# Lacadame/DiffSci

Measured on AMD Instinct MI355X. Metric: samples/sec (50-step Karras Heun), PUNetG 64ch 128x128, higher is better.
Workload: dtype f32 (3x3 convs: fp16 hi+lo split, 3 fp16 MFMA products, fp32 accumulate); 1 GPU; PUNetG 64-base-ch, 1x128x128 fields, batch 64 per GPU, 50-step Heun deterministic sampler (99 network evaluations); global_batch=64, parallelism=dp1 (batch shards, all-gather of samples), world_size=1, backend=none (one process), hipgraph=True

## Files before the change

diffsci_amd/_native.py:

```python
import ctypes
import os
from ctypes import POINTER, Structure, c_char_p, c_float, c_int, c_longlong, c_size_t, c_uint32, c_uint64, c_void_p

_HERE = os.path.dirname(os.path.abspath(__file__))
LIB_PATH = os.environ.get("DIFFSCI_HIP_LIB") or os.path.join(_HERE, "_lib", "libdiffsci_hip.so")

ABI_VERSION = 4
DS_IN_NETWORK, DS_IN_SCORE, DS_IN_DRIFT, DS_IN_FLOW = 0, 1, 2, 3
DS_LOAD_PLAIN, DS_LOAD_MAXPOOL2, DS_LOAD_UPSAMPLE2, DS_LOAD_AVGPOOL2 = 0, 1, 2, 3
DS_PAD_CIRCULAR = 16
DS_RES1_UPSAMPLED = 32


class EvalCoef(Structure):
    _fields_ = [("c_out", c_float), ("c_skip", c_float), ("sigma_sq", c_float),
                ("neg_mult", c_float), ("neg_lang", c_float), ("guidance", c_float),
                ("one_minus_guidance", c_float), ("input_kind", c_int), ("stochastic", c_int),
                ("scaled", c_int), ("scale", c_float), ("scale_mult", c_float), ("next_scale", c_float), ("xin_copies", c_int),
                ("nonfinite", c_void_p)]


class NativeLibraryError(RuntimeError):
    pass


_P = c_void_p
_PROTOS = {
    "ds_version": (c_int, []),
    "ds_last_error": (c_char_p, []),
    "ds_device_info": (c_int, [POINTER(c_int), POINTER(c_int), ctypes.c_char_p, c_int]),
    "ds_karras_scale": (c_int, [_P, _P, c_float, c_size_t, _P]),
    "ds_karras_drift": (c_int, [_P, _P, _P, _P, POINTER(EvalCoef), c_size_t, _P]),
    "ds_karras_score": (c_int, [_P, _P, _P, _P, POINTER(EvalCoef), c_size_t, _P]),
    "ds_philox_normal": (c_int, [_P, _P, c_uint64, c_size_t, _P]),
    "ds_karras_euler": (c_int, [_P, _P, _P, _P, _P, POINTER(EvalCoef), c_float, c_float,
                                _P, _P, c_uint64, c_float, c_float, c_size_t, _P]),
    "ds_karras_heun": (c_int, [_P, _P, _P, _P, _P, POINTER(EvalCoef), _P, _P, POINTER(EvalCoef),
                               c_float, c_float, c_size_t, _P]),
    "ds_karras_churn": (c_int, [_P, _P, _P, _P, _P, c_uint64, c_float, c_float, c_float, c_float, c_int, c_size_t, _P]),
    "ds_karras_denoiser": (c_int, [_P, _P, _P, _P, c_float, c_float, _P, _P, c_int, c_size_t, _P]),
    "ds_inorm_silu": (c_int, [_P, _P, _P, _P, c_int, c_int, c_int, c_float, c_int, _P]),
    "ds_conv2d_packed_floats": (c_size_t, [c_int, c_int, c_int]),
    "ds_conv2d_pack_weights": (c_int, [_P, _P, c_int, c_int, c_int, _P]),
    "ds_conv2d": (c_int, [_P, _P, _P, _P, _P, c_int, _P, _P, c_int, c_int, c_int, c_int, c_int,
                          c_int, c_int, _P]),
    "ds_conv2d_x6_packed_bytes": (c_size_t, [c_int, c_int]),
    "ds_conv2d_x6_pack_weights": (c_int, [_P, _P, c_int, c_int, _P]),
    "ds_conv2d_x6": (c_int, [_P, _P, _P, _P, _P, c_int, _P, _P, c_int, c_int, c_int, c_int, c_int, c_int, _P]),
    "ds_conv2d_h3_packed_bytes": (c_size_t, [c_int, c_int]),
    "ds_conv2d_h3_pack_weights": (c_int, [_P, _P, c_int, c_int, c_int, _P]),
    "ds_conv2d_h3": (c_int, [_P, _P, _P, c_int, _P, _P, c_int, _P, _P, c_int, c_int, c_int, c_int, c_int, c_int, _P, _P, _P, _P, _P]),
    "ds_absmax_rows": (c_int, [_P, _P, c_int, c_size_t, c_size_t, _P]),
    "ds_amax_merge": (c_int, [_P, _P, _P, c_int, _P]),
    "ds_absmax_channels": (c_int, [_P, _P, _P, _P, _P, c_int, c_int, c_size_t, c_int, _P]),
    "ds_input_amax": (c_int, [_P, c_int, c_int, _P, _P, _P, c_int, c_int, c_size_t, c_int, _P]),
    "ds_fill_u32": (c_int, [_P, c_uint32, c_size_t, _P]),
    "ds_conv2d_h3_up_supported": (c_int, [c_int, c_int]),
    "ds_conv2d_h3_up_packed_bytes": (c_size_t, [c_int, c_int]),
    "ds_conv2d_h3_up_pack_weights": (c_int, [_P, _P, c_int, c_int, c_int, _P]),
    "ds_conv2d_h3_up": (c_int, [_P, _P, _P, c_int, _P, _P, c_int, _P, _P, c_int, c_int, c_int, c_int, c_int, c_int, _P, _P, _P, _P, _P]),
    "ds_table_apply_images": (c_int, [_P, _P, _P, c_int, c_int, c_int, c_int, _P]),
    "ds_conv2d_h3_up_img": (c_int, [_P, _P, _P, c_int, _P, _P, c_int, _P, _P, c_int, c_int, c_int, c_int, c_int, _P, _P, _P]),
    "ds_conv_tile_count": (c_int, [c_int, c_int]),
    "ds_inorm_table": (c_int, [_P, _P, _P, _P, c_int, c_int, c_int, c_int, c_float, c_int, _P]),
    "ds_gnorm1_table": (c_int, [_P, _P, c_int, c_int, _P, c_int, c_int, _P, _P, _P, _P, c_int, c_int, c_longlong,
                                c_float, c_int, _P]),
    "ds_gnorm1_stats_tiles": (c_int, [_P, _P, c_int, c_int, _P, c_int, c_int, c_int, c_longlong, c_float, c_int, _P]),
    "ds_conv2d_direct": (c_int, [_P, _P, _P, _P, c_int, c_int, c_int, c_int, c_int, c_int, _P]),
    "ds_conv3d_direct": (c_int, [_P, _P, _P, _P, _P, c_int, _P, _P, c_int, c_int, c_int, c_int, c_int, c_int, c_int, _P]),
    "ds_volume_to_slices": (c_int, [_P, _P, c_int, c_int, c_int, c_size_t, c_int, c_int, c_int, _P]),
    "ds_slices_to_volume": (c_int, [_P, _P, _P, _P, c_int, c_int, c_int, c_size_t, c_int, _P]),
    "ds_conv_images_bytes": (c_size_t, [c_int, c_int, c_int, c_int]),
    "ds_inorm_silu_images_supported": (c_int, [c_int, c_int]),
    "ds_inorm_silu_images": (c_int, [_P, _P, _P, _P, c_int, c_int, c_int, c_int, c_float, c_int, _P]),
    "ds_conv2d_h3_img": (c_int, [_P, _P, _P, c_int, _P, _P, c_int, _P, _P, c_int, c_int, c_int, c_int, c_int, c_int, _P, _P, _P]),
    "ds_gnorm1_apply_images": (c_int, [_P, _P, _P, _P, _P, _P, _P, c_int, c_int, c_int, c_int, c_int, c_int, c_int, _P]),
    "ds_volume_stat_tiles": (c_int, [c_int, c_size_t]),
    "ds_volume_to_slices_act": (c_int, [_P, _P, _P, c_int, c_int, c_int, c_size_t, c_int, _P]),
    "ds_wrap_pad_slices": (c_int, [_P, c_int, c_int, c_int, c_size_t, _P]),
    "ds_slices_to_volume_stats": (c_int, [_P, _P, _P, _P, _P, c_int, c_int, c_int, c_size_t, c_int, _P]),
    "ds_slice_tables": (c_int, [_P, _P, _P, _P, c_int, c_int, c_int, c_int, c_longlong, c_float, c_int, c_int, _P]),
    "ds_avgpool3d": (c_int, [_P, _P, c_int, c_int, c_int, c_int, _P]),
    "ds_upsample3d": (c_int, [_P, _P, c_int, c_int, c_int, c_int, _P]),
    "ds_avgpool3d_f": (c_int, [_P, _P, c_int, c_int, c_int, c_int, c_int, _P]),
    "ds_upsample_f": (c_int, [_P, _P, c_int, c_int, c_int, c_int, c_int, c_int, _P]),
    "ds_maxpool_f": (c_int, [_P, _P, c_int, c_int, c_int, c_int, c_int, c_int, _P]),
    "ds_cornerpool_f": (c_int, [_P, _P, _P, _P, c_int, c_int, c_int, c_int, c_int, c_int, c_int, c_int, c_int, _P]),
    "ds_conv1x1_h3_packed_bytes": (c_size_t, [c_int, c_int]),
    "ds_conv1x1_h3_pack_weights": (c_int, [_P, _P, c_int, c_int, c_int, _P]),
    "ds_conv1x1_h3": (c_int, [_P, _P, _P, c_int, _P, _P, c_int, _P, _P, c_int, c_int, c_int, c_int, c_int, c_int, _P, _P, _P, c_int, _P]),
    "ds_attention": (c_int, [_P, _P, c_int, c_int, c_int, _P]),
    "ds_attention_generic": (c_int, [_P, _P, c_int, c_int, c_int, _P]),
    "ds_attention_h3": (c_int, [_P, _P, c_int, c_int, c_int, _P, _P, _P]),
    "ds_attention_h3_workspace_bytes": (c_size_t, [c_int, c_int, c_int]),
    "ds_attention_h3_ws": (c_int, [_P, _P, _P, c_int, c_int, c_int, _P, _P, _P]),
    "ds_attention_h3_heads_workspace_bytes": (c_size_t, [c_int, c_int, c_int, c_int]),
    "ds_attention_h3_heads": (c_int, [_P, _P, _P, c_int, c_int, c_int, c_int, _P, _P, _P]),
    "ds_attention_heads_generic": (c_int, [_P, _P, c_int, c_int, c_int, c_int, _P]),
    "ds_token_l2_normalize": (c_int, [_P, c_int, c_int, c_int, c_int, c_int, c_float, c_float, _P]),
    "ds_linear": (c_int, [_P, _P, _P, _P, c_int, c_int, c_int, c_int, _P]),
    "ds_fourier_features": (c_int, [_P, _P, _P, _P, c_int, c_int, c_int, _P]),
    "ds_fourier_channels": (c_int, [_P, _P, _P, c_int, c_int, c_int, c_size_t, _P]),
    "ds_gnorm1_workspace_bytes": (c_size_t, [c_int]),
    "ds_gnorm1_stats": (c_int, [_P, _P, _P, c_int, c_int, c_int, c_float, c_int, _P]),
    "ds_groupnorm_stats": (c_int, [_P, _P, _P, c_int, c_int, c_int, c_int, c_float, _P]),
    "ds_groupnorm_apply": (c_int, [_P, _P, _P, _P, _P, c_int, c_int, c_int, c_int, c_int, _P, _P]),
    "ds_groupnorm_stats_tiles": (c_int, [_P, _P, c_int, c_int, c_int, c_int, c_longlong, c_float, _P]),
    "ds_groupnorm_table": (c_int, [_P, _P, _P, _P, _P, c_int, c_int, c_int, c_int, c_longlong, c_float, _P]),
    "ds_gnorm1_apply": (c_int, [_P, _P, _P, _P, _P, _P, _P, c_int, c_int, c_int, c_int, c_int, c_int, c_int, _P]),
    "ds_gnorm1_apply_poolf": (c_int, [_P, _P, _P, _P, _P, _P, _P, c_int, c_int, c_int, c_int, c_int, c_int, c_int, _P]),
    "ds_concat2": (c_int, [_P, _P, _P, c_int, c_size_t, c_size_t, _P]),
    "ds_add_act": (c_int, [_P, _P, _P, c_int, c_int, c_int, c_int, _P]),
    "ds_mask_blend": (c_int, [_P, _P, _P, _P, c_size_t, c_int, _P]),
    "ds_axpby": (c_int, [_P, _P, c_float, _P, c_float, c_size_t, _P]),
    "ds_div_scalar": (c_int, [_P, _P, c_float, c_size_t, _P]),
    "ds_batchnorm_eval": (c_int, [_P, _P, _P, _P, _P, _P, c_float, c_float, c_int, c_int, c_int, c_int, c_size_t, _P]),
    "ds_lerp_stack": (c_int, [_P, _P, _P, c_int, c_size_t, _P]),
    "ds_add": (c_int, [_P, _P, _P, c_size_t, _P]),
    "ds_token_layernorm": (c_int, [_P, _P, _P, _P, _P, _P, c_int, c_int, c_int, c_int, c_float, _P, _P]),
    "ds_token_gate": (c_int, [_P, _P, _P, _P, c_int, c_int, c_int, c_int, _P]),
    "ds_silu_amax": (c_int, [_P, _P, c_int, c_size_t, _P, _P]),
    "ds_patch_embed": (c_int, [_P, _P, _P, _P, c_int, c_int, c_int, c_int, c_int, c_int, _P]),
    "ds_patch_unembed": (c_int, [_P, _P, _P, _P, c_int, c_int, c_int, c_int, c_int, c_int, _P]),
    "ds_graph_begin_capture": (c_int, [_P]),
    "ds_graph_end_capture": (c_int, [_P, POINTER(_P), POINTER(c_int)]),
    "ds_graph_launch": (c_int, [_P, _P]),
    "ds_graph_destroy": (c_int, [_P]),
}

_lib = None


def exported_symbols():
    return sorted(_PROTOS)


def lib():
    global _lib
    if _lib is not None:
        return _lib
    if not os.path.exists(LIB_PATH):
        raise NativeLibraryError(
            f"{LIB_PATH} is missing: diffsci_amd has no CPU or PyTorch fallback. "
# ... 23 lines not shown
```

diffsci_amd/csrc/ds_conv1h.hip:

```cpp
#include "ds_common.h"
#include "ds_conv_epilogue.h"

namespace {

using ds_epi::f32x16;
typedef unsigned u32x4 __attribute__((ext_vector_type(4)));
typedef _Float16 f16x8 __attribute__((ext_vector_type(8)));
typedef _Float16 f16x2 __attribute__((ext_vector_type(2)));
typedef const __attribute__((address_space(1))) float* gfloat_ptr;
typedef const __attribute__((address_space(1))) char* gchar_ptr;
typedef float f32x2 __attribute__((ext_vector_type(2)));
typedef const __attribute__((address_space(1))) f32x2* gfloat2_ptr;

constexpr int COT = 64, NT = 256, KC = 16;
constexpr int NPOS = 256;
constexpr int XBUF_VEC = 2 * 2 * NPOS;
constexpr int WSLAB_VEC = 2 * 2 * COT;
constexpr int NXB = 3, NWS = 3;
constexpr int RING_BYTES = (NXB * XBUF_VEC + NWS * WSLAB_VEC) * 16;
constexpr int EPI_BYTES = 4 * 64 * 2 * 32 * 4;
constexpr int STAGE_BYTES = RING_BYTES > EPI_BYTES ? RING_BYTES : EPI_BYTES;
constexpr int LDS_BYTES = STAGE_BYTES + 128 * 4;
constexpr int TWO_RING_BYTES = (NXB * XBUF_VEC + NWS * 2 * WSLAB_VEC) * 16;
constexpr int TWO_EPI_BYTES = 8 * 64 * 2 * 32 * 4;
static_assert(TWO_EPI_BYTES >= TWO_RING_BYTES, "bias / shift rows behind the larger of the two");
constexpr int LDS_BYTES_TWO = TWO_EPI_BYTES + 2 * 128 * 4;
constexpr int NXCD = 8;

struct Conv1hArgs {
  float* out;
  const float* in;
  const u32x4* wp;
  const float* bias;
  const float* shift;
  const float* res1;
  const float* res2;
  float* tile_stats;
  int res1_up;
  const unsigned* in_amax;
  unsigned* out_amax;
  int wshift;
  int amax_split;
  int shift_stride;
  int B, Cin, Cout, H, W, Hin, Win;
  int tiles_x, tiles_y, n_cot, n_chunks;
  int n_cot_wg;
  unsigned n_blocks;
};

__device__ __forceinline__ void split2(float a, float b, unsigned& hi, unsigned& lo) {
  f16x2 h = {(_Float16)a, (_Float16)b};
  unsigned hp = __builtin_bit_cast(unsigned, h);
  asm volatile("" : "+v"(hp));
  const f16x2 hq = __builtin_bit_cast(f16x2, hp);
  f16x2 l = {(_Float16)(a - (float)hq[0]), (_Float16)(b - (float)hq[1])};
  hi = hp;
  lo = __builtin_bit_cast(unsigned, l);
}

__device__ __forceinline__ void step_barrier() {
  asm volatile("s_waitcnt lgkmcnt(0)\n\ts_barrier" ::: "memory");
}

template <int MODE, bool W16, bool TWO = false>
__global__ __launch_bounds__(TWO ? 2 * NT : NT, 2) void k_conv1h(const Conv1hArgs a) {
  constexpr int TW = W16 ? 16 : 32, TH = W16 ? 16 : 8;
  constexpr int COTS = TWO ? 2 : 1;
  constexpr int KR = TWO ? KC / 2 : KC;
  extern __shared__ __attribute__((aligned(16))) unsigned char smem[];
  u32x4* Xs = reinterpret_cast<u32x4*>(smem);
  u32x4* Ws = Xs + NXB * XBUF_VEC;
  float* BS = reinterpret_cast<float*>(smem + (TWO ? TWO_EPI_BYTES : STAGE_BYTES));
  const int tid = threadIdx.x;
  const int lane = tid & 63;
  const int wv = __builtin_amdgcn_readfirstlane(tid >> 6);
  const int cw = TWO ? wv >> 2 : 0;
  const int wq = wv & 3;
  const int pix = tid & (NT - 1);
  const int li = lane & 31, lh = lane >> 5;
// ... 101 lines not shown
  w_fetch(W1, n > 1 ? 1 : 0);
  x_fetch(R1, n > 1 ? 1 : 0);
  __builtin_amdgcn_sched_barrier(0);
  ascale = ds_epi::act_scale_of(amax_bits, a.wshift);
  w_store(W0, 0);
  x_store(R0, 0);
  ds_epi::commit_bias_shift(BS, bias_shift, COTS);
  __syncthreads();

  int buf = 0;
  auto step = [&](float (&Ra)[KR], u32x4& Wa, float (&Rb)[KR], u32x4& Wb, int g) {
    const int gf = g + 2 < n ? g + 2 : n - 1;
    w_fetch(Wa, gf);
    x_fetch(Ra, gf);
    mma(g % NWS, buf);
    const int nb = buf == NXB - 1 ? 0 : buf + 1;
    w_store(Wb, (g + 1) % NWS);
    x_store(Rb, nb);
    buf = nb;
    step_barrier();
  };
  int g = 0;
  for (; g + 1 < n; g += 2) {
    step(R0, W0, R1, W1, g);
    step(R1, W1, R0, W0, g + 1);
  }
  if (g < n) step(R0, W0, R1, W1, g);
  __syncthreads();

  {
    ds_epi::Args e;
    e.out = a.out; e.bias = a.bias; e.shift = a.shift; e.res1 = a.res1; e.res2 = a.res2; e.res1_up = a.res1_up;
    e.unscale = ds_epi::unscale_from_in(ascale.in_scale, a.wshift); e.shift_stride = a.shift_stride;
    e.out_amax = a.out_amax ? a.out_amax + b + ((a.amax_split > 0 && (cot + cw) * COT >= a.amax_split) ? a.B : 0) : nullptr;
    e.b = b; e.co_base = (cot + cw) * COT; e.y0 = y0 + (W16 ? 4 : 2) * wq; e.x0 = x0;
    e.Cout = a.Cout; e.H = a.H; e.W = a.W;
    e.tile_stats = a.tile_stats; e.tile = ty * a.tiles_x + tx; e.ntiles = a.tiles_x * a.tiles_y;
    float* tile = reinterpret_cast<float*>(smem) + wv * (64 * 2 * 32);
    ds_epi::store_tile<W16>(acc, tile, BS + 128 * cw, e);
    if (a.tile_stats) {
      __syncthreads();
      if constexpr (TWO) {
        if (tid < 128) {
          e.co_base = (cot + (tid >> 6)) * COT;
          ds_epi::store_tile_stats(reinterpret_cast<const float*>(smem) + (tid >> 6) * 4 * (64 * 2 * 32), 64 * 2 * 32, e, tid & 63);
        }
      } else {
        ds_epi::store_tile_stats(reinterpret_cast<const float*>(smem), 64 * 2 * 32, e);
      }
    }
  }
}

__global__ void k_pack1h(_Float16* packed, const float* __restrict__ w, int Cout, int Cin, int n_chunks, float scale,
                         size_t total) {
  size_t i = (size_t)blockIdx.x * blockDim.x + threadIdx.x;
  if (i >= total) return;
  size_t t = i;
  const int c8 = t % 8; t /= 8;
  const int co64 = t % COT; t /= COT;
  const int h = t % 2; t /= 2;
  const int piece = t % 2; t /= 2;
  const int chunk = t % n_chunks; t /= n_chunks;
  const int cot = (int)t;
  const int co = cot * COT + co64, ci = chunk * KC + 8 * h + c8;
  float v = 0.f;
  if (co < Cout && ci < Cin) v = w[(size_t)co * Cin + ci] * scale;
  const _Float16 hi = (_Float16)v;
  const _Float16 lo = (_Float16)(v - (float)hi);
  packed[i] = piece == 0 ? hi : lo;
}

inline int conv1h_two() {
  static const int v = [] { const char* e = getenv("DS_CONV1_TWO"); return e ? atoi(e) : 1; }();
  return v;
}
inline long long conv1h_two_min() {
  static const long long v = [] { const char* e = getenv("DS_CONV1_TWO_MIN"); return e ? atoll(e) : 256ll; }();
  return v;
}

template <int MODE, bool W16>
int launch_conv1h(Conv1hArgs a, hipStream_t s) {
  const int two = conv1h_two();
  if (a.n_cot % 2 == 0 && ((two == 1 && (long long)a.n_blocks / 2 >= conv1h_two_min()) || two == 2)) {
    const int rc = ds::ensure_dynamic_lds<&k_conv1h<MODE, W16, true>>((int)(LDS_BYTES_TWO), "hipFuncSetAttribute(conv1h two)");
    if (rc != DS_OK) return rc;
    a.n_cot_wg = a.n_cot / 2;
    a.n_blocks /= 2;
    hipLaunchKernelGGL((k_conv1h<MODE, W16, true>), dim3(a.n_blocks), dim3(2 * NT), LDS_BYTES_TWO, s, a);
    DS_CHECK_LAUNCH("ds_conv1x1_h3");
    return DS_OK;
  }
  {
    const int rc = ds::ensure_dynamic_lds<&k_conv1h<MODE, W16>>((int)(LDS_BYTES), "hipFuncSetAttribute(conv1h)");
    if (rc != DS_OK) return rc;
  }
  a.n_cot_wg = a.n_cot;
  hipLaunchKernelGGL((k_conv1h<MODE, W16>), dim3(a.n_blocks), dim3(NT), LDS_BYTES, s, a);
  DS_CHECK_LAUNCH("ds_conv1x1_h3");
  return DS_OK;
}

}

extern "C" {

size_t ds_conv1x1_h3_packed_bytes(int Cout, int Cin) {
  if (Cout <= 0 || Cin <= 0) return 0;
  const size_t n_cot = (Cout + COT - 1) / COT, n_chunks = (Cin + KC - 1) / KC;
  return n_cot * n_chunks * (size_t)WSLAB_VEC * 16;
}

int ds_conv1x1_h3_pack_weights(void* packed, const float* w, int Cout, int Cin, int wshift, void* stream) {
  DS_REQUIRE(packed && w, DS_ERR_NULL, "ds_conv1x1_h3_pack_weights: NULL pointer");
  DS_REQUIRE(Cout > 0 && Cin > 0, DS_ERR_SHAPE, "ds_conv1x1_h3_pack_weights: Cout=%d Cin=%d", Cout, Cin);
  DS_REQUIRE(wshift >= -40 && wshift <= 40, DS_ERR_SHAPE, "ds_conv1x1_h3_pack_weights: wshift %d out of range", wshift);
  const int n_chunks = (Cin + KC - 1) / KC;
  const size_t total = ds_conv1x1_h3_packed_bytes(Cout, Cin) / 2;
  hipLaunchKernelGGL(k_pack1h, dim3((unsigned)((total + 255) / 256)), dim3(256), 0, ds::as_stream(stream),
                     reinterpret_cast<_Float16*>(packed), w, Cout, Cin, n_chunks, ldexpf(1.0f, wshift), total);
  DS_CHECK_LAUNCH("ds_conv1x1_h3_pack_weights");
  return DS_OK;
}

int ds_conv1x1_h3(float* out, const float* in, const void* w_packed, int wshift, const float* bias, const float* shift,
                  int shift_stride, const float* res1, const float* res2, int B, int Cin, int Cout, int H, int W,
                  int load_mode, float* tile_stats, const unsigned* in_amax, unsigned* out_amax, int amax_split, void* stream) {
  DS_REQUIRE(out && in && w_packed, DS_ERR_NULL, "ds_conv1x1_h3: NULL pointer");
  DS_REQUIRE(B >= 0 && Cin > 0 && Cout > 0 && H > 0 && W > 0, DS_ERR_SHAPE,
             "ds_conv1x1_h3: bad shape B=%d Cin=%d Cout=%d H=%d W=%d", B, Cin, Cout, H, W);
  DS_REQUIRE(load_mode == DS_LOAD_PLAIN || load_mode == DS_LOAD_UPSAMPLE2 || load_mode == DS_LOAD_AVGPOOL2,
             DS_ERR_UNSUPPORTED, "ds_conv1x1_h3: load_mode %d", load_mode);
  DS_REQUIRE(load_mode != DS_LOAD_UPSAMPLE2 || (H % 2 == 0 && W % 2 == 0), DS_ERR_SHAPE,
             "ds_conv1x1_h3: UPSAMPLE2 needs even output H, W (got %d x %d)", H, W);
  DS_REQUIRE(shift == nullptr || shift_stride == 0 || shift_stride >= Cout, DS_ERR_SHAPE,
             "ds_conv1x1_h3: shift_stride %d < Cout %d", shift_stride, Cout);
  DS_REQUIRE((reinterpret_cast<uintptr_t>(w_packed) & 15u) == 0, DS_ERR_SHAPE, "ds_conv1x1_h3: w_packed must be 16-byte aligned");
  DS_REQUIRE(load_mode != DS_LOAD_AVGPOOL2 || (reinterpret_cast<uintptr_t>(in) & 7u) == 0, DS_ERR_SHAPE,
             "ds_conv1x1_h3: AVGPOOL2 input must be 8-byte aligned");
  DS_REQUIRE(wshift >= -40 && wshift <= 40, DS_ERR_SHAPE, "ds_conv1x1_h3: wshift %d out of range", wshift);
  DS_REQUIRE(amax_split >= 0 && amax_split % COT == 0, DS_ERR_SHAPE, "ds_conv1x1_h3: amax_split %d must be a multiple of 64", amax_split);
  if (B == 0) return DS_OK;
  Conv1hArgs a;
  a.out = out; a.in = in; a.wp = reinterpret_cast<const u32x4*>(w_packed); a.bias = bias; a.shift = shift;
  a.res1 = res1; a.res2 = res2; a.shift_stride = shift_stride; a.tile_stats = tile_stats; a.res1_up = 0;
  a.wshift = wshift; a.in_amax = in_amax; a.out_amax = out_amax; a.amax_split = amax_split;
  a.B = B; a.Cin = Cin; a.Cout = Cout; a.H = H; a.W = W;
  a.Hin = load_mode == DS_LOAD_AVGPOOL2 ? 2 * H : (load_mode == DS_LOAD_UPSAMPLE2 ? H / 2 : H);
  a.Win = load_mode == DS_LOAD_AVGPOOL2 ? 2 * W : (load_mode == DS_LOAD_UPSAMPLE2 ? W / 2 : W);
  DS_REQUIRE((long long)a.Hin * a.Win < (1ll << 29), DS_ERR_SHAPE, "ds_conv1x1_h3: a channel plane exceeds 2^29 floats");
  const long long pad32 = (long long)((W + 31) / 32 * 32) * ((H + 7) / 8 * 8);
  const long long pad16 = (long long)((W + 15) / 16 * 16) * ((H + 15) / 16 * 16);
  const bool w16 = pad16 < pad32;
  const int TW = w16 ? 16 : 32, TH = w16 ? 16 : 8;
  a.tiles_x = (W + TW - 1) / TW; a.tiles_y = (H + TH - 1) / TH;
  a.n_cot = (Cout + COT - 1) / COT;
  a.n_chunks = (Cin + KC - 1) / KC;
  const long long blocks = (long long)B * a.tiles_y * a.tiles_x * a.n_cot;
  DS_REQUIRE(blocks > 0 && blocks < (1ll << 31), DS_ERR_SHAPE, "ds_conv1x1_h3: grid of %lld workgroups is out of range", blocks);
  a.n_blocks = (unsigned)blocks;
  hipStream_t s = ds::as_stream(stream);
  if (w16) {
    if (load_mode == DS_LOAD_PLAIN) return launch_conv1h<DS_LOAD_PLAIN, true>(a, s);
    if (load_mode == DS_LOAD_UPSAMPLE2) return launch_conv1h<DS_LOAD_UPSAMPLE2, true>(a, s);
    return launch_conv1h<DS_LOAD_AVGPOOL2, true>(a, s);
  }
  if (load_mode == DS_LOAD_PLAIN) return launch_conv1h<DS_LOAD_PLAIN, false>(a, s);
  if (load_mode == DS_LOAD_UPSAMPLE2) return launch_conv1h<DS_LOAD_UPSAMPLE2, false>(a, s);
  return launch_conv1h<DS_LOAD_AVGPOOL2, false>(a, s);
}

}
```

diffsci_amd/ops.py:

```python
import ctypes

import torch

from . import _native as N
from ._native import EvalCoef


def require_device(t, what="tensor"):
    if not isinstance(t, torch.Tensor):
        raise TypeError(f"{what} must be a torch.Tensor")
    if not t.is_cuda:
        raise RuntimeError(
            f"{what} lives on {t.device}: diffsci_amd computes only on an AMD GPU through "
            "libdiffsci_hip.so (there is no CPU path; move the module and inputs to 'cuda').")
    if t.dtype != torch.float32:
        raise TypeError(f"{what} has dtype {t.dtype}; the HIP path is fp32 only")
    if t.device.index != torch.cuda.current_device():
        raise RuntimeError(f"{what} lives on {t.device} but the current device is cuda:{torch.cuda.current_device()}: "
                           "wrap the call in `with torch.cuda.device(tensor.device):` (KarrasModule / SIModule / the "
                           "networks do this for their own entry points)")


def on_device_of(t):
    return torch.cuda.device(t.device)
# ... 858 lines not shown
def conv_tile_count(H, W):
    return N.lib().ds_conv_tile_count(int(H), int(W))


def table_channels(C):
    return (C + 15) // 16 * 16


def inorm_table(tile_stats, w, b, kind, count, eps=1e-5, out=None):
    B, C, nt, _ = tile_stats.shape
    if out is None:
        out = torch.empty((B, table_channels(C), 4), dtype=torch.float32, device=tile_stats.device)
    elif tuple(out.shape) != (B, table_channels(C), 4):
        raise ValueError(f"table must be {(B, table_channels(C), 4)}")
    N.check(N.lib().ds_inorm_table(_p(out), _p(tile_stats), _p(w), _p(b), B, C, nt, int(count), float(eps), int(kind),
                                   _stream()), "ds_inorm_table")
    return out


def gnorm1_table(stats_a, w, b, kind, count, stats_b=None, film=None, eps=1e-5, out=None):
    B, Ca, nta, _ = stats_a.shape
    Cb, ntb = (0, 0) if stats_b is None else (stats_b.shape[1], stats_b.shape[2])
    C = Ca + Cb
    if out is None:
        out = torch.empty((B, table_channels(C), 4), dtype=torch.float32, device=stats_a.device)
    elif tuple(out.shape) != (B, table_channels(C), 4):
        raise ValueError(f"table must be {(B, table_channels(C), 4)}")
    f1 = f2 = None
    stride = 0
    if film is not None:
        if film.dim() != 2 or film.shape[1] != 2 * C or film.shape[0] not in (1, B):
            raise ValueError("film must be [1 or B, 2C]")
        require_device(film, "film")
        stride = 0 if film.shape[0] == 1 else 2 * C
        f1, f2 = film.data_ptr(), film.data_ptr() + 4 * C
    N.check(N.lib().ds_gnorm1_table(_p(out), _p(stats_a), Ca, nta, _p(stats_b), Cb, ntb, _p(w), _p(b), f1, f2, stride,
                                    B, int(count), float(eps), int(kind), _stream()), "ds_gnorm1_table")
    return out


def gnorm1_stats_tiles(stats_a, kind, count, stats_b=None, eps=1e-5, stats=None):
    require_device(stats_a, "stats_a")
    B, Ca, nta, _ = stats_a.shape
    Cb, ntb = (0, 0) if stats_b is None else (stats_b.shape[1], stats_b.shape[2])
    if stats is None:
        stats = torch.empty((B, 2), dtype=torch.float32, device=stats_a.device)
    elif tuple(stats.shape) != (B, 2):
        raise ValueError(f"stats must be {(B, 2)}")
    N.check(N.lib().ds_gnorm1_stats_tiles(_p(stats), _p(stats_a), Ca, nta, _p(stats_b), Cb, ntb, B, int(count), float(eps),
                                          int(kind), _stream()), "ds_gnorm1_stats_tiles")
    return stats


def conv2d(x, w_packed, Cout, ks, bias=None, shift=None, res1=None, res2=None,
           load_mode=N.DS_LOAD_PLAIN, out=None, kind="fp32", wshift=0, prenorm=None, tile_stats=None, circular=False,
           res1_upsampled=False, w_up=None, up_wshift=0, tap_offset=None, in_amax=None, out_amax=None, amax_split=0):
    B, Cin, Hin, Win = x.shape
    if load_mode in (N.DS_LOAD_MAXPOOL2, N.DS_LOAD_AVGPOOL2):
        if Hin % 2 or Win % 2:
            raise ValueError("pooling load needs even input H, W")
        if (load_mode == N.DS_LOAD_AVGPOOL2) != (kind == "fp16x3" and ks == 1):
            raise ValueError("load modes: AVGPOOL2 is for the fp16x3 1x1 kernel, MAXPOOL2 for the others")
        H, W = Hin // 2, Win // 2
    elif load_mode == N.DS_LOAD_UPSAMPLE2:
        H, W = Hin * 2, Win * 2
    else:
        H, W = Hin, Win
    if out is None:
        out = torch.empty((B, Cout, H, W), dtype=torch.float32, device=x.device)
    elif tuple(out.shape) != (B, Cout, H, W):
        raise ValueError(f"out has shape {tuple(out.shape)}, expected {(B, Cout, H, W)}")
    expect = {"bf16x6": lambda: N.lib().ds_conv2d_x6_packed_bytes(Cout, Cin) // 4,
              "fp16x3": lambda: (N.lib().ds_conv2d_h3_packed_bytes if ks == 3 else
                                 N.lib().ds_conv1x1_h3_packed_bytes)(Cout, Cin) // 4,
              "fp32": lambda: N.lib().ds_conv2d_packed_floats(Cout, Cin, ks)}[kind]()
    if w_packed.numel() != expect or (kind == "bf16x6" and ks != 3) or ks not in (1, 3):
        raise ValueError("packed weight size does not match (Cout, Cin, ks)")
    stride = 0
    if shift is not None:
        if shift.dim() != 2 or shift.shape[1] != Cout or shift.shape[0] not in (1, B):
            raise ValueError(f"shift must be [1 or B, Cout]; got {tuple(shift.shape)}")
        stride = 0 if shift.shape[0] == 1 else Cout
    if res1_upsampled:
        if kind != "fp16x3" or ks != 3 or res1 is None or H % 2 or W % 2 or tuple(res1.shape) != (B, Cout, H // 2, W // 2):
            raise ValueError("res1_upsampled: fp16x3 3x3 convolution with res1 of shape [B, Cout, H/2, W/2]")
    for r in ((res2,) if res1_upsampled else (res1, res2)):
        if r is not None and tuple(r.shape) != (B, Cout, H, W):
            raise ValueError("residual shape mismatch")
    if bias is not None and bias.numel() != Cout:
        raise ValueError("bias must have Cout entries")
    if (prenorm is not None or tile_stats is not None) and kind != "fp16x3":
        raise ValueError("prenorm / tile_stats are features of the fp16x3 kernels")
    pin = pout = None
    if kind == "fp16x3":
        pin = _in_amax(x, in_amax, B, raw=prenorm is None)
        if amax_split and (ks != 1 or amax_split % 64):
            raise ValueError("amax_split: the fp16x3 1x1 convolution, a multiple of 64")
        pout = _pi(out_amax, 2 * B if amax_split else B, "out_amax")
    elif out_amax is not None:
        raise ValueError("out_amax is a feature of the fp16x3 kernels (use absmax_rows on the result)")
    if circular and ks == 3 and kind != "fp16x3":
        raise NotImplementedError("periodic padding is implemented in the fp16x3 convolution only")
    if prenorm is not None and (ks != 3 or tuple(prenorm.shape) != (B, table_channels(Cin), 4)):
        raise ValueError(f"prenorm must be [B, ceil16(Cin), 4] on a 3x3 convolution; got {tuple(prenorm.shape)}")
    if tile_stats is not None and tuple(tile_stats.shape) != (B, Cout, conv_tile_count(H, W), 4):
        raise ValueError(f"tile_stats must be {(B, Cout, conv_tile_count(H, W), 4)}; got {tuple(tile_stats.shape)}")
    tap = 0
    if tap_offset is not None and tuple(tap_offset) != (0, 0):
        oy, ox = (int(v) for v in tap_offset)
        if kind != "fp16x3" or ks != 3 or not (-8 <= oy <= 7 and -8 <= ox <= 7):
            raise ValueError("tap_offset: fp16x3 3x3 convolution, offsets in [-8, 7]")
        tap = ((oy & 15) << 8) | ((ox & 15) << 12)
        w_up = None
    if kind == "fp16x3" and ks == 1:
        N.check(N.lib().ds_conv1x1_h3(_p(out), _p(x), _p(w_packed), int(wshift), _p(bias), _p(shift), stride,
                                      _p(res1), _p(res2), B, Cin, Cout, H, W, load_mode, _p(tile_stats), pin, pout,
                                      int(amax_split), _stream()), "ds_conv1x1_h3")
    elif kind == "fp16x3" and load_mode == N.DS_LOAD_UPSAMPLE2 and w_up is not None \
            and N.lib().ds_conv2d_h3_up_supported(Hin, Win):
        if w_up.numel() != N.lib().ds_conv2d_h3_up_packed_bytes(Cout, Cin) // 4:
            raise ValueError("w_up size does not match (Cout, Cin)")
        N.check(N.lib().ds_conv2d_h3_up(_p(out), _p(x), _p(w_up), int(up_wshift), _p(bias), _p(shift), stride,
                                        _p(res1), _p(res2), B, Cin, Cout, Hin, Win,
                                        (N.DS_PAD_CIRCULAR if circular else 0) | (N.DS_RES1_UPSAMPLED if res1_upsampled else 0),
                                        _p(prenorm), _p(tile_stats), pin, pout, _stream()), "ds_conv2d_h3_up")
    elif kind == "fp16x3":
        N.check(N.lib().ds_conv2d_h3(_p(out), _p(x), _p(w_packed), int(wshift), _p(bias), _p(shift), stride,
                                     _p(res1), _p(res2), B, Cin, Cout, H, W,
                                     load_mode | tap | (N.DS_PAD_CIRCULAR if circular else 0) | (N.DS_RES1_UPSAMPLED if res1_upsampled else 0),
                                     _p(prenorm), _p(tile_stats), pin, pout,
                                     _stream()), "ds_conv2d_h3")
    elif kind == "bf16x6":
        N.check(N.lib().ds_conv2d_x6(_p(out), _p(x), _p(w_packed), _p(bias), _p(shift), stride, _p(res1),
                                     _p(res2), B, Cin, Cout, H, W, load_mode, _stream()), "ds_conv2d_x6")
    else:
        N.check(N.lib().ds_conv2d(_p(out), _p(x), _p(w_packed), _p(bias), _p(shift), stride, _p(res1), _p(res2),
                                  B, Cin, Cout, H, W, ks, load_mode, _stream()), "ds_conv2d")
    return out


def conv_images_floats(B, C, H, W):
    return N.lib().ds_conv_images_bytes(int(B), int(C), int(H), int(W)) // 4


def inorm_silu_images_supported(H, W):
    return bool(N.lib().ds_inorm_silu_images_supported(int(H), int(W)))


def inorm_silu_images(x, w, b, kind, eps=1e-5, out=None):
    require_device(x, "x")
    B, C, H, W = x.shape
    n = conv_images_floats(B, C, H, W)
    if out is None:
        out = torch.empty(n, dtype=torch.float32, device=x.device)
    elif out.numel() != n:
        raise ValueError("images buffer size does not match x")
    if w is not None and (w.numel() != C or b.numel() != C):
        raise ValueError("norm affine parameters must have C entries")
    N.check(N.lib().ds_inorm_silu_images(_p(out), _p(x), _p(w), _p(b), B, C, H, W, float(eps), int(kind), _stream()),
            "ds_inorm_silu_images")
    return out


def conv_img(images, pw, B, Cin, H, W, bias=None, shift=None, res1=None, res2=None, tile_stats=None, out=None,
             res1_upsampled=False, out_amax=None):
    require_device(images, "images")
    if pw.kind != "fp16x3" or pw.ks != 3 or pw.subs is not None:
# ... 384 lines not shown
```

include/diffsci_hip.h:

```cpp
#ifndef DIFFSCI_HIP_H
#define DIFFSCI_HIP_H

#include <stddef.h>
#include <stdint.h>

#ifdef __cplusplus
extern "C" {
#endif

typedef enum ds_status {
  DS_OK = 0,
  DS_ERR_SHAPE = -1,
  DS_ERR_NULL = -2,
  DS_ERR_HIP = -3,
  DS_ERR_UNSUPPORTED = -4
} ds_status;

int ds_version(void);
const char* ds_last_error(void);
int ds_device_info(int* cu_count, int* lds_bytes_per_cu, char* arch_name, int arch_name_len);

typedef struct ds_eval_coef {
  float c_out;
  float c_skip;
// ... 103 lines not shown
                    const unsigned* in_amax, unsigned* out_amax, void* stream);
int ds_conv2d_h3_up_img(float* out, const void* images, const void* w_packed, int wshift, const float* bias,
                        const float* shift, int shift_stride, const float* res1, const float* res2,
                        int B, int Cin, int Cout, int Hl, int Wl, float* tile_stats, unsigned* out_amax, void* stream);


int ds_inorm_table(float* table, const float* tile_stats, const float* w, const float* b, int B, int C, int ntiles,
                   int count, float eps, int kind, void* stream);

int ds_gnorm1_table(float* table, const float* stats_a, int Ca, int ntiles_a, const float* stats_b, int Cb,
                    int ntiles_b, const float* w, const float* b, const float* film_scale, const float* film_shift,
                    int film_stride, int B, long long count, float eps, int kind, void* stream);
int ds_gnorm1_stats_tiles(float* stats, const float* stats_a, int Ca, int ntiles_a, const float* stats_b, int Cb,
                          int ntiles_b, int B, long long count, float eps, int kind, void* stream);

int ds_conv2d_direct(float* out, const float* in, const float* w, const float* bias, int B, int Cin, int Cout,
                     int H, int W, int circular, void* stream);

int ds_conv3d_direct(float* out, const float* in, const float* w, const float* bias, const float* shift,
                     int shift_stride, const float* res1, const float* res2, int B, int Cin, int Cout, int D, int H,
                     int W, int load_mode, void* stream);

int ds_volume_to_slices(float* slices, const float* x, int B, int C, int D, size_t HW, int depth_mode, int circular,
                        int pad , void* stream);
int ds_slices_to_volume(float* y, const float* slices, const float* res1, const float* res2, int B, int C, int D,
                        size_t HW, int pad, void* stream);

int ds_volume_stat_tiles(int D, size_t HW);
int ds_volume_to_slices_act(float* slices, const float* x, const float* table, int B, int C, int D, size_t HW, int circular,
                            void* stream);
int ds_wrap_pad_slices(float* slices, int B, int C, int D, size_t HW, void* stream);
int ds_slices_to_volume_stats(float* y, const float* slices, const float* res1, const float* res2, float* stats, int B, int C,
                              int D, size_t HW, int pad, void* stream);
int ds_slice_tables(float* table, const float* tile_stats, const float* w, const float* b, int B, int C, int D, int ntiles,
                    long long count, float eps, int kind, int circular, void* stream);

int ds_avgpool3d(float* out, const float* x, int planes, int Do, int Ho, int Wo, void* stream);
int ds_upsample3d(float* out, const float* x, int planes, int Di, int Hi, int Wi, void* stream);

int ds_avgpool3d_f(float* out, const float* x, int planes, int Di, int Hi, int Wi, int factor, void* stream);
int ds_upsample_f(float* out, const float* x, int planes, int Di, int Hi, int Wi, int factor, int volume, void* stream);

int ds_maxpool_f(float* out, const float* x, int planes, int Di, int Hi, int Wi, int factor, int volume, void* stream);

int ds_cornerpool_f(float* out, const float* x, const float* te, unsigned* out_amax, int B, int C, int Di, int Hi, int Wi,
                    int factor, int volume, int x_batch, int te_batch, void* stream);

size_t ds_conv1x1_h3_packed_bytes(int Cout, int Cin);
int ds_conv1x1_h3_pack_weights(void* packed, const float* w, int Cout, int Cin, int wshift, void* stream);
int ds_conv1x1_h3(float* out, const float* in, const void* w_packed, int wshift, const float* bias,
                  const float* shift, int shift_stride, const float* res1, const float* res2,
                  int B, int Cin, int Cout, int H, int W, int load_mode, float* tile_stats,
                  const unsigned* in_amax, unsigned* out_amax, int amax_split, void* stream);

int ds_attention(float* out, const float* qkv, int B, int E, int L, void* stream);

int ds_attention_generic(float* out, const float* qkv, int B, int E, int L, void* stream);

int ds_token_l2_normalize(float* x, int B, int Ctot, int c0, int C, int L, float eps, float gain, void* stream);

int ds_attention_h3(float* out, const float* qkv, int B, int E, int L, const unsigned* in_amax, unsigned* out_amax, void* stream);
size_t ds_attention_h3_workspace_bytes(int B, int E, int L);
int ds_attention_h3_ws(float* out, const float* qkv, void* workspace, int B, int E, int L, const unsigned* in_amax,
                       unsigned* out_amax, void* stream);
size_t ds_attention_h3_heads_workspace_bytes(int B, int E, int heads, int L);
int ds_attention_h3_heads(float* out, const float* qkv, void* workspace, int B, int E, int heads, int L, const unsigned* in_amax,
                          unsigned* out_amax, void* stream);
int ds_attention_heads_generic(float* out, const float* qkv, int B, int E, int heads, int L, void* stream);

int ds_linear(float* y, const float* x, const float* w, const float* b, int M, int K, int N, int act, void* stream);

int ds_fourier_features(float* out, const float* t, const float* W, const float* add, int add_rows,
                        int M, int half, void* stream);

int ds_fourier_channels(float* out, const float* x, const float* W, int B, int C, int D, size_t HW, void* stream);


size_t ds_gnorm1_workspace_bytes(int B);
int ds_gnorm1_stats(float* stats, void* workspace, const float* x, int B, int C, int HW, float eps, int kind,
                    void* stream);

int ds_groupnorm_stats(float* stats, void* workspace, const float* x, int B, int C, int G, int N, float eps, void* stream);
int ds_groupnorm_apply(float* out, const float* x, const float* stats, const float* w, const float* b, int B, int C, int G, int N,
                       int act, unsigned* out_amax, void* stream);
int ds_groupnorm_stats_tiles(float* stats, const float* tile_stats, int B, int C, int G, int ntiles, long long count, float eps,
                             void* stream);
int ds_groupnorm_table(float* table, const float* tile_stats, const float* stats, const float* w, const float* b, int B, int C,
                       int G, int ntiles, long long count, float eps, void* stream);

int ds_gnorm1_apply(float* out, const float* x, const float* stats, const float* w, const float* b,
                    const float* film_scale, const float* film_shift, int film_stride,
                    int B, int C, int H, int W, int kind, int pool, void* stream);

int ds_gnorm1_apply_poolf(float* out, const float* x, const float* stats, const float* w, const float* b,
                          const float* film_scale, const float* film_shift, int film_stride,
                          int B, int C, int H, int W, int kind, int factor, void* stream);

int ds_concat2(float* out, const float* a, const float* b, int B, size_t na, size_t nb, void* stream);

int ds_add_act(float* out, const float* a, const float* add, int add_rows, int M, int N, int act, void* stream);

int ds_mask_blend(float* out, const float* x, const float* y, const float* mask, size_t n_per_sample, int B,
                  void* stream);

int ds_axpby(float* out, const float* x, float a, const float* y, float b, size_t n, void* stream);
int ds_div_scalar(float* out, const float* x, float s, size_t n, void* stream);
// ... 34 lines not shown
```

Measured before the change: 83.21 samples/s.

## Add four-output-tile 1x1 conv kernel sharing each input tile across channel tiles

Adds a k_conv1h4 variant of the fp16x3 1x1 convolution. Each 512-thread workgroup computes four 64-channel output tiles from one staged input tile, where the existing kernels compute one or two, so the input fetch, hi/lo split and LDS staging are amortised over more output channels. It is selected by default when there are at least three channel tiles, padding waste is small and enough blocks remain, and an env var plus an explicit route API allow forcing either path. The cost is fewer blocks per launch, more accumulators per thread and higher LDS use, which can lower occupancy and parallelism on mid-sized layers.

```diff
diff --git a/diffsci_amd/_native.py b/diffsci_amd/_native.py
--- a/diffsci_amd/_native.py
+++ b/diffsci_amd/_native.py
@@ -9,6 +9,7 @@
 DS_IN_NETWORK, DS_IN_SCORE, DS_IN_DRIFT, DS_IN_FLOW = 0, 1, 2, 3
 DS_LOAD_PLAIN, DS_LOAD_MAXPOOL2, DS_LOAD_UPSAMPLE2, DS_LOAD_AVGPOOL2 = 0, 1, 2, 3
 DS_PAD_CIRCULAR = 16
+DS_CONV1_ROUTE_AUTO, DS_CONV1_ROUTE_TILES, DS_CONV1_ROUTE_ALL = -1, 0, 1
 DS_RES1_UPSAMPLED = 32
 
 
@@ -89,6 +90,8 @@
     "ds_conv1x1_h3_packed_bytes": (c_size_t, [c_int, c_int]),
     "ds_conv1x1_h3_pack_weights": (c_int, [_P, _P, c_int, c_int, c_int, _P]),
     "ds_conv1x1_h3": (c_int, [_P, _P, _P, c_int, _P, _P, c_int, _P, _P, c_int, c_int, c_int, c_int, c_int, c_int, _P, _P, _P, c_int, _P]),
+    "ds_conv1x1_h3_route": (c_int, [_P, _P, _P, c_int, _P, _P, c_int, _P, _P, c_int, c_int, c_int, c_int, c_int, c_int, _P, _P, _P, c_int,
+                                    c_int, _P, _P]),
     "ds_attention": (c_int, [_P, _P, c_int, c_int, c_int, _P]),
     "ds_attention_generic": (c_int, [_P, _P, c_int, c_int, c_int, _P]),
     "ds_attention_h3": (c_int, [_P, _P, c_int, c_int, c_int, _P, _P, _P]),
diff --git a/diffsci_amd/csrc/ds_conv1h.hip b/diffsci_amd/csrc/ds_conv1h.hip
--- a/diffsci_amd/csrc/ds_conv1h.hip
+++ b/diffsci_amd/csrc/ds_conv1h.hip
@@ -25,6 +25,12 @@
 constexpr int TWO_EPI_BYTES = 8 * 64 * 2 * 32 * 4;
 static_assert(TWO_EPI_BYTES >= TWO_RING_BYTES, "bias / shift rows behind the larger of the two");
 constexpr int LDS_BYTES_TWO = TWO_EPI_BYTES + 2 * 128 * 4;
+constexpr int ALL_COTS = 4;
+constexpr int ALL_RING_BYTES = (NXB * XBUF_VEC + NWS * ALL_COTS * WSLAB_VEC) * 16;
+constexpr int ALL_EPI_BYTES = 8 * 64 * 2 * 32 * 4;
+static_assert(ALL_EPI_BYTES >= ALL_RING_BYTES, "bias / shift rows behind the larger of the two");
+constexpr int LDS_BYTES_ALL = ALL_EPI_BYTES + ALL_COTS * 128 * 4;
+static_assert(LDS_BYTES_ALL <= 160 * 1024, "LDS of a CU");
 constexpr int NXCD = 8;
 
 struct Conv1hArgs {
@@ -232,6 +238,206 @@
   }
 }
 
+template <int MODE, bool W16>
+__global__ __launch_bounds__(2 * NT, 2) void k_conv1h4(const Conv1hArgs a) {
+  constexpr int TW = W16 ? 16 : 32, TH = W16 ? 16 : 8;
+  constexpr int KR = KC / 2;
+  extern __shared__ __attribute__((aligned(16))) unsigned char smem[];
+  u32x4* Xs = reinterpret_cast<u32x4*>(smem);
+  u32x4* Ws = Xs + NXB * XBUF_VEC;
+  float* BS = reinterpret_cast<float*>(smem + ALL_EPI_BYTES);
+  const int tid = threadIdx.x;
+  const int lane = tid & 63;
+  const int wv = __builtin_amdgcn_readfirstlane(tid >> 6);
+  const int cw = wv >> 2;
+  const int wq = wv & 3;
+  const int pix = tid & (NT - 1);
+  const int li = lane & 31, lh = lane >> 5;
+
+  unsigned bid;
+  {
+    const unsigned x = blockIdx.x % NXCD, k = blockIdx.x / NXCD;
+    const unsigned per = a.n_blocks / NXCD, rem = a.n_blocks % NXCD;
+    bid = x * per + (x < rem ? x : rem) + k;
+  }
+  const int cot = (int)(bid % a.n_cot_wg) * ALL_COTS; bid /= a.n_cot_wg;
+  const int tx = bid % a.tiles_x; bid /= a.tiles_x;
+  const int ty = bid % a.tiles_y; bid /= a.tiles_y;
+  const int b = bid;
+  const int x0 = tx * TW, y0 = ty * TH;
+  const int HWin = a.Hin * a.Win;
+  const int n = a.n_chunks;
+
+  const int gy = y0 + (W16 ? pix >> 4 : pix >> 5), gx = x0 + (W16 ? pix & 15 : pix & 31);
+  const bool ok = gy < a.H && gx < a.W;
+  unsigned off;
+  if (MODE == DS_LOAD_PLAIN) off = gy * a.Win + gx;
+  else if (MODE == DS_LOAD_UPSAMPLE2) off = (gy >> 1) * a.Win + (gx >> 1);
+  else off = (2 * gy) * a.Win + 2 * gx;
+  if (!ok) off = 0;
+  const unsigned offb = off * 4u, rowb = (unsigned)a.Win * 4u;
+  const float* in_b = a.in + (size_t)b * a.Cin * HWin;
+  const int ct0 = cot + 2 * cw, ct1 = ct0 + 1;
+  const u32x4* wp0 = a.wp + (size_t)(ct0 < a.n_cot ? ct0 : a.n_cot - 1) * n * WSLAB_VEC;
+  const u32x4* wp1 = a.wp + (size_t)(ct1 < a.n_cot ? ct1 : a.n_cot - 1) * n * WSLAB_VEC;
+  ds_epi::ActScale ascale;
+
+  auto x_fetch = [&](float (&R)[KR], int chunk) {
+    const int cbase = chunk * KC + KR * cw;
+    unsigned ob = offb;
+    asm volatile("" : "+v"(ob));
+#pragma unroll
+    for (int c = 0; c < KR; ++c) {
+      const int ch = cbase + c < a.Cin ? cbase + c : a.Cin - 1;
+      gchar_ptr p = (gchar_ptr)(in_b + (size_t)ch * HWin);
+      asm volatile("" : "+s"(p));
+      if (MODE == DS_LOAD_AVGPOOL2) {
+        const f32x2 t0 = *(gfloat2_ptr)(p + ob);
+        const f32x2 t1 = *(gfloat2_ptr)(p + (ob + rowb));
+        R[c] = (((t0.x + t0.y) + t1.x) + t1.y) / 4.0f;
+      } else {
+        R[c] = *(gfloat_ptr)(p + ob);
+      }
+    }
+  };
+  auto x_store = [&](const float (&R)[KR], int buf) {
+    u32x4* xb = Xs + buf * XBUF_VEC;
+    u32x4 qh, ql;
+#pragma unroll
+    for (int k = 0; k < 4; ++k) {
+      unsigned ph, pl;
+      split2(R[2 * k] * ascale.in_scale, R[2 * k + 1] * ascale.in_scale, ph, pl);
+      qh[k] = ph; ql[k] = pl;
+    }
+    xb[cw * NPOS + pix] = qh;
+    xb[(2 + cw) * NPOS + pix] = ql;
+  };
+  auto w_fetch = [&](u32x4 (&Wr)[2], int chunk) {
+    Wr[0] = wp0[(size_t)chunk * WSLAB_VEC + pix];
+    Wr[1] = wp1[(size_t)chunk * WSLAB_VEC + pix];
+  };
+  auto w_store = [&](const u32x4 (&Wr)[2], int slot) {
+    Ws[(slot * ALL_COTS + 2 * cw) * WSLAB_VEC + pix] = Wr[0];
+    Ws[(slot * ALL_COTS + 2 * cw + 1) * WSLAB_VEC + pix] = Wr[1];
+  };
+
+  f32x16 acc[2][2][2];
+#pragma unroll
+  for (int j = 0; j < 2; ++j)
+#pragma unroll
+    for (int m = 0; m < 2; ++m)
+#pragma unroll
+      for (int r = 0; r < 2; ++r)
+#pragma unroll
+        for (int q = 0; q < 16; ++q) acc[j][m][r][q] = 0.f;
+
+  auto mma = [&](int slot, int buf) {
+    const u32x4* xb = Xs + buf * XBUF_VEC;
+    f16x8 fb[2][2];
+#pragma unroll
+    for (int p = 0; p < 2; ++p)
+#pragma unroll
+      for (int r = 0; r < 2; ++r) fb[p][r] = *reinterpret_cast<const f16x8*>(&xb[(p * 2 + lh) * NPOS + (2 * wq + r) * 32 + li]);
+    constexpr int PA[3] = {1, 0, 0};
+    constexpr int PB[3] = {0, 1, 0};
+#pragma unroll
+    for (int j = 0; j < 2; ++j) {
+      const u32x4* wb = Ws + (slot * ALL_COTS + 2 * cw + j) * WSLAB_VEC;
+      f16x8 fa[2][2];
+#pragma unroll
+      for (int p = 0; p < 2; ++p)
+#pragma unroll
+        for (int m = 0; m < 2; ++m) fa[p][m] = *reinterpret_cast<const f16x8*>(&wb[(p * 2 + lh) * COT + 32 * m + li]);
+#pragma unroll
+      for (int t = 0; t < 3; ++t)
+#pragma unroll
+        for (int m = 0; m < 2; ++m)
+#pragma unroll
+          for (int r = 0; r < 2; ++r)
+            acc[j][m][r] = __builtin_amdgcn_mfma_f32_32x32x16_f16(fa[PA[t]][m], fb[PB[t]][r], acc[j][m][r], 0, 0, 0);
+    }
+  };
+
+  float R0[KR], R1[KR];
+  u32x4 W0[2], W1[2];
+  const float bias_shift = ds_epi::fetch_bias_shift(a.bias, a.shift, a.shift_stride, b, (cot + (tid >> 7)) * COT, a.Cout, ALL_COTS);
+  __builtin_amdgcn_sched_barrier(0);
+  const unsigned amax_bits = ds_epi::act_bits(a.in_amax, b);
+  w_fetch(W0, 0);
+  x_fetch(R0, 0);
+  w_fetch(W1, n > 1 ? 1 : 0);
+  x_fetch(R1, n > 1 ? 1 : 0);
+  __builtin_amdgcn_sched_barrier(0);
+  ascale = ds_epi::act_scale_of(amax_bits, a.wshift);
+  w_store(W0, 0);
+  x_store(R0, 0);
+  ds_epi::commit_bias_shift(BS, bias_shift, ALL_COTS);
+  __syncthreads();
+
+  int buf = 0;
+  auto step = [&](float (&Ra)[KR], u32x4 (&Wa)[2], float (&Rb)[KR], u32x4 (&Wb)[2], int g) {
+    const int gf = g + 2 < n ? g + 2 : n - 1;
+    w_fetch(Wa, gf);
+    x_fetch(Ra, gf);
+    mma(g % NWS, buf);
+    const int nb = buf == NXB - 1 ? 0 : buf + 1;
+    w_store(Wb, (g + 1) % NWS);
+    x_store(Rb, nb);
+    buf = nb;
+    step_barrier();
+  };
+  int g = 0;
+  for (; g + 1 < n; g += 2) {
+    step(R0, W0, R1, W1, g);
+    step(R1, W1, R0, W0, g + 1);
+  }
+  if (g < n) step(R0, W0, R1, W1, g);
+  __syncthreads();
+
+  {
+    ds_epi::Args e;
+    e.out = a.out; e.bias = a.bias; e.shift = a.shift; e.res1 = a.res1; e.res2 = a.res2; e.res1_up = a.res1_up;
+    e.unscale = ds_epi::unscale_from_in(ascale.in_scale, a.wshift); e.shift_stride = a.shift_stride;
+    e.b = b; e.y0 = y0 + (W16 ? 4 : 2) * wq; e.x0 = x0;
+    e.Cout = a.Cout; e.H = a.H; e.W = a.W;
+    e.tile_stats = a.tile_stats; e.tile = ty * a.tiles_x + tx; e.ntiles = a.tiles_x * a.tiles_y;
+    float* tile = reinterpret_cast<float*>(smem) + wv * (64 * 2 * 32);
+#pragma unroll
+    for (int t = 0; t < 2; ++t) {
+      const int ct = ct0 + t;
+      if (t == 1 && a.tile_stats) __syncthreads();
+      if (ct < a.n_cot) {
+        e.out_amax = a.out_amax ? a.out_amax + b + ((a.amax_split > 0 && ct * COT >= a.amax_split) ? a.B : 0) : nullptr;
+        const float* bs = BS + 128 * (2 * cw + t);
+#pragma unroll
+        for (int m = 0; m < 2; ++m)
+#pragma unroll
+          for (int q = 0; q < 16; ++q) {
+            const int co = 32 * m + (q & 3) + 8 * (q >> 2) + 4 * lh;
+            const float bsv = bs[co] + bs[64 + co];
+#pragma unroll
+            for (int r = 0; r < 2; ++r) tile[(co * 2 + r) * 32 + li] = __builtin_fmaf(acc[t][m][r][q], e.unscale, bsv);
+          }
+#pragma unroll
+        for (int m = 0; m < 2; ++m) {
+          e.co_base = ct * COT + 32 * m;
+          ds_epi::store_tile_rows<W16, 1, false>(tile + m * (32 * 2 * 32), e, ds_epi::Residuals<0>{});
+        }
+      }
+      if (a.tile_stats) {
+        __syncthreads();
+        if (tid < 128) {
+          ds_epi::Args es = e;
+          const int m = (tid >> 5) & 1;
+          es.co_base = (cot + 2 * (tid >> 6) + t) * COT + 32 * m;
+          ds_epi::store_tile_stats(reinterpret_cast<const float*>(smem) + (tid >> 6) * 4 * (64 * 2 * 32) + m * (32 * 2 * 32),
+                                   64 * 2 * 32, es, tid & 31);
+        }
+      }
+    }
+  }
+}
+
 __global__ void k_pack1h(_Float16* packed, const float* __restrict__ w, int Cout, int Cin, int n_chunks, float scale,
                          size_t total) {
   size_t i = (size_t)blockIdx.x * blockDim.x + threadIdx.x;
@@ -260,8 +466,31 @@
   return v;
 }
 
+inline int conv1h_all() {
+  static const int v = [] { const char* e = getenv("DS_CONV1_ALL"); return e ? atoi(e) : 1; }();
+  return v;
+}
+inline long long conv1h_all_min() {
+  static const long long v = [] { const char* e = getenv("DS_CONV1_ALL_MIN"); return e ? atoll(e) : 256ll; }();
+  return v;
+}
+
 template <int MODE, bool W16>
-int launch_conv1h(Conv1hArgs a, hipStream_t s) {
+int launch_conv1h(Conv1hArgs a, int route, int* taken, hipStream_t s) {
+  const int all = route == DS_CONV1_ROUTE_AUTO ? conv1h_all() : (route == DS_CONV1_ROUTE_ALL ? 2 : 0);
+  const int groups = (a.n_cot + ALL_COTS - 1) / ALL_COTS;
+  const long long all_blocks = (long long)(a.n_blocks / a.n_cot) * groups;
+  const bool all_fits = 8 * (groups * ALL_COTS - a.n_cot) <= groups * ALL_COTS && all_blocks >= conv1h_all_min();
+  if (a.n_cot >= 3 && a.W % 4 == 0 && ((all == 1 && all_fits) || all == 2)) {
+    const int rc = ds::ensure_dynamic_lds<&k_conv1h4<MODE, W16>>((int)(LDS_BYTES_ALL), "hipFuncSetAttribute(conv1h all)");
+    if (rc != DS_OK) return rc;
+    a.n_cot_wg = groups;
+    a.n_blocks = (unsigned)all_blocks;
+    hipLaunchKernelGGL((k_conv1h4<MODE, W16>), dim3(a.n_blocks), dim3(2 * NT), LDS_BYTES_ALL, s, a);
+    DS_CHECK_LAUNCH("ds_conv1x1_h3");
+    if (taken) *taken = ALL_COTS;
+    return DS_OK;
+  }
   const int two = conv1h_two();
   if (a.n_cot % 2 == 0 && ((two == 1 && (long long)a.n_blocks / 2 >= conv1h_two_min()) || two == 2)) {
     const int rc = ds::ensure_dynamic_lds<&k_conv1h<MODE, W16, true>>((int)(LDS_BYTES_TWO), "hipFuncSetAttribute(conv1h two)");
@@ -270,6 +499,7 @@
     a.n_blocks /= 2;
     hipLaunchKernelGGL((k_conv1h<MODE, W16, true>), dim3(a.n_blocks), dim3(2 * NT), LDS_BYTES_TWO, s, a);
     DS_CHECK_LAUNCH("ds_conv1x1_h3");
+    if (taken) *taken = 2;
     return DS_OK;
   }
   {
@@ -279,6 +509,7 @@
   a.n_cot_wg = a.n_cot;
   hipLaunchKernelGGL((k_conv1h<MODE, W16>), dim3(a.n_blocks), dim3(NT), LDS_BYTES, s, a);
   DS_CHECK_LAUNCH("ds_conv1x1_h3");
+  if (taken) *taken = 1;
   return DS_OK;
 }
 
@@ -307,6 +538,17 @@
 int ds_conv1x1_h3(float* out, const float* in, const void* w_packed, int wshift, const float* bias, const float* shift,
                   int shift_stride, const float* res1, const float* res2, int B, int Cin, int Cout, int H, int W,
                   int load_mode, float* tile_stats, const unsigned* in_amax, unsigned* out_amax, int amax_split, void* stream) {
+  return ds_conv1x1_h3_route(out, in, w_packed, wshift, bias, shift, shift_stride, res1, res2, B, Cin, Cout, H, W, load_mode,
+                             tile_stats, in_amax, out_amax, amax_split, DS_CONV1_ROUTE_AUTO, nullptr, stream);
+}
+
+int ds_conv1x1_h3_route(float* out, const float* in, const void* w_packed, int wshift, const float* bias, const float* shift,
+                        int shift_stride, const float* res1, const float* res2, int B, int Cin, int Cout, int H, int W,
+                        int load_mode, float* tile_stats, const unsigned* in_amax, unsigned* out_amax, int amax_split,
+                        int route, int* route_taken, void* stream) {
+  DS_REQUIRE(route == DS_CONV1_ROUTE_AUTO || route == DS_CONV1_ROUTE_TILES || route == DS_CONV1_ROUTE_ALL, DS_ERR_UNSUPPORTED,
+             "ds_conv1x1_h3: route %d", route);
+  if (route_taken) *route_taken = 0;
   DS_REQUIRE(out && in && w_packed, DS_ERR_NULL, "ds_conv1x1_h3: NULL pointer");
   DS_REQUIRE(B >= 0 && Cin > 0 && Cout > 0 && H > 0 && W > 0, DS_ERR_SHAPE,
              "ds_conv1x1_h3: bad shape B=%d Cin=%d Cout=%d H=%d W=%d", B, Cin, Cout, H, W);
@@ -342,13 +584,13 @@
   a.n_blocks = (unsigned)blocks;
   hipStream_t s = ds::as_stream(stream);
   if (w16) {
-    if (load_mode == DS_LOAD_PLAIN) return launch_conv1h<DS_LOAD_PLAIN, true>(a, s);
-    if (load_mode == DS_LOAD_UPSAMPLE2) return launch_conv1h<DS_LOAD_UPSAMPLE2, true>(a, s);
-    return launch_conv1h<DS_LOAD_AVGPOOL2, true>(a, s);
-  }
-  if (load_mode == DS_LOAD_PLAIN) return launch_conv1h<DS_LOAD_PLAIN, false>(a, s);
-  if (load_mode == DS_LOAD_UPSAMPLE2) return launch_conv1h<DS_LOAD_UPSAMPLE2, false>(a, s);
-  return launch_conv1h<DS_LOAD_AVGPOOL2, false>(a, s);
-}
-
-}
+    if (load_mode == DS_LOAD_PLAIN) return launch_conv1h<DS_LOAD_PLAIN, true>(a, route, route_taken, s);
+    if (load_mode == DS_LOAD_UPSAMPLE2) return launch_conv1h<DS_LOAD_UPSAMPLE2, true>(a, route, route_taken, s);
+    return launch_conv1h<DS_LOAD_AVGPOOL2, true>(a, route, route_taken, s);
+  }
+  if (load_mode == DS_LOAD_PLAIN) return launch_conv1h<DS_LOAD_PLAIN, false>(a, route, route_taken, s);
+  if (load_mode == DS_LOAD_UPSAMPLE2) return launch_conv1h<DS_LOAD_UPSAMPLE2, false>(a, route, route_taken, s);
+  return launch_conv1h<DS_LOAD_AVGPOOL2, false>(a, route, route_taken, s);
+}
+
+}
diff --git a/diffsci_amd/ops.py b/diffsci_amd/ops.py
--- a/diffsci_amd/ops.py
+++ b/diffsci_amd/ops.py
@@ -934,9 +934,14 @@
     return stats
 
 
+conv1x1_route = None
+conv1x1_route_taken = 0
+
+
 def conv2d(x, w_packed, Cout, ks, bias=None, shift=None, res1=None, res2=None,
            load_mode=N.DS_LOAD_PLAIN, out=None, kind="fp32", wshift=0, prenorm=None, tile_stats=None, circular=False,
-           res1_upsampled=False, w_up=None, up_wshift=0, tap_offset=None, in_amax=None, out_amax=None, amax_split=0):
+           res1_upsampled=False, w_up=None, up_wshift=0, tap_offset=None, in_amax=None, out_amax=None, amax_split=0,
+           route=None):
     B, Cin, Hin, Win = x.shape
     if load_mode in (N.DS_LOAD_MAXPOOL2, N.DS_LOAD_AVGPOOL2):
         if Hin % 2 or Win % 2:
@@ -994,7 +999,16 @@
             raise ValueError("tap_offset: fp16x3 3x3 convolution, offsets in [-8, 7]")
         tap = ((oy & 15) << 8) | ((ox & 15) << 12)
         w_up = None
-    if kind == "fp16x3" and ks == 1:
+    if route is None:
+        route = conv1x1_route
+    if kind == "fp16x3" and ks == 1 and route is not None:
+        global conv1x1_route_taken
+        taken = ctypes.c_int(0)
+        N.check(N.lib().ds_conv1x1_h3_route(_p(out), _p(x), _p(w_packed), int(wshift), _p(bias), _p(shift), stride,
+                                            _p(res1), _p(res2), B, Cin, Cout, H, W, load_mode, _p(tile_stats), pin, pout,
+                                            int(amax_split), int(route), ctypes.addressof(taken), _stream()), "ds_conv1x1_h3_route")
+        conv1x1_route_taken = taken.value
+    elif kind == "fp16x3" and ks == 1:
         N.check(N.lib().ds_conv1x1_h3(_p(out), _p(x), _p(w_packed), int(wshift), _p(bias), _p(shift), stride,
                                       _p(res1), _p(res2), B, Cin, Cout, H, W, load_mode, _p(tile_stats), pin, pout,
                                       int(amax_split), _stream()), "ds_conv1x1_h3")
diff --git a/include/diffsci_hip.h b/include/diffsci_hip.h
--- a/include/diffsci_hip.h
+++ b/include/diffsci_hip.h
@@ -179,6 +179,12 @@
                   const float* shift, int shift_stride, const float* res1, const float* res2,
                   int B, int Cin, int Cout, int H, int W, int load_mode, float* tile_stats,
                   const unsigned* in_amax, unsigned* out_amax, int amax_split, void* stream);
+enum { DS_CONV1_ROUTE_AUTO = -1, DS_CONV1_ROUTE_TILES = 0, DS_CONV1_ROUTE_ALL = 1 };
+int ds_conv1x1_h3_route(float* out, const float* in, const void* w_packed, int wshift, const float* bias,
+                        const float* shift, int shift_stride, const float* res1, const float* res2,
+                        int B, int Cin, int Cout, int H, int W, int load_mode, float* tile_stats,
+                        const unsigned* in_amax, unsigned* out_amax, int amax_split, int route, int* route_taken,
+                        void* stream);
 
 int ds_attention(float* out, const float* qkv, int B, int E, int L, void* stream);
 
```

After: 82.84 samples/s. About the same (-0.4%).
